# Gepetto/mpc-interface

Measured on AMD Instinct MI355X. Metric: QP assemblies/sec (P,q,G,h), biped N=16 batched, higher is better.
Workload: dtype f64; 1 GPU; C2 biped LIPM N=16 no=36 nc=76, per-instance (A,B)/given/aim, K1 on chip; batch_per_gpu=4096, global_batch=4096, streams=2

## Files before the change

mpc-interface_amd/csrc/resident.hip:

```cpp
#ifdef __HIPCC_RTC__
using __hip_internal::int32_t;
using __hip_internal::int64_t;
using __hip_internal::uint32_t;
using __hip_internal::uint64_t;
typedef unsigned long uintptr_t;
#else
#include <hip/hip_runtime.h>
#include <stdint.h>
#endif

#include "device_prims.h"
#include "plan_dev.h"
#ifdef MPCASM_SPEC
#include "plan_spec.h"
#endif
#ifndef __HIPCC_RTC__
#include "kernels.h"
#endif

namespace mpcasm {

#ifndef __HIPCC_RTC__
extern int g_phase_mask;
extern int g_resident_per_cu;
#endif

namespace {

constexpr int NT = RS_NT;
constexpr int MW = RS_NW;
constexpr int WT = NT - MW * 64;
constexpr int AXMAX = RS_AXMAX;
constexpr int RR_WORDS = RS_RR_WORDS;
constexpr int RR_COMPACT = 4;
static_assert(RS_DIAG_MAX == 2, "the per-column diagonal table holds two terms");

__host__ __device__ inline int even_up_i(int x) { return (x + 1) & ~1; }

constexpr int GU = 6;
template <class PlanT>
__host__ __device__ inline int resident_g_mode(const PlanT& p) {
  if (p.csc_gnnz != 0 || p.csc_pnnz != 0) return 3;
  if (!p.rr_packed) return 0;
  return p.rs_ngdesc != 0 ? 2 : 1;
}
static_assert(GU == RS_GDESC_PIECES && WT == RS_GDESC_THREADS, "descriptor table of G");

template <class PlanT>
__host__ __device__ inline int resident_v_doubles(const PlanT& p) {
  return (p.rs_vrow0 + p.rtot) * p.rs_ldv + 16;
}

struct ResidentLayout {
  int v, pl, ql, dvec, dcoef, dpar, img, ab, streams, ints, total_doubles;
  int ldp;
  int p_direct;
  int i_rr, i_meta, i_wtrip, i_split, i_lti, i_abmeta, i_gdesc, i_gfix, i_rrwin, i_cscp;
};

template <class PlanT>
__host__ __device__ inline ResidentLayout resident_layout(const PlanT& p) {
  ResidentLayout L;
  L.ldp = even_up_i(p.no);
  int o = 0;
  L.v = o;      o += resident_v_doubles(p);
  L.pl = o;
  L.ql = o;     o += L.ldp;
  L.dvec = o;   o += 2 * L.ldp;
  L.dcoef = o;  o += RS_DIAG_MAX * L.ldp;
  L.dpar = o;   o += RS_DIAG_MAX * L.ldp;
  L.img = o;    o += 2 * p.rs_img;
  L.ab = o;     o += 2 * p.rs_ab;
  L.streams = o; o += 2 * (MAX_SOURCES + 3);
  L.ints = o;
  int i = 0;
  L.i_rr = i;    i += p.nc * (p.rr_packed ? RR_COMPACT : RR_WORDS);
  L.i_meta = i;  i += p.rs_nchunk * 64 * 2;
  L.i_abmeta = i; i += p.rs_ab * 2 * 2;
  L.i_gdesc = i;  i += resident_g_mode(p) == 2 ? GU * WT * 2 : (resident_g_mode(p) == 3 ? 2 * p.csc_gnnz : 0);
  L.i_gfix = i;   i += resident_g_mode(p) == 2 && p.rs_ngfix != 0 ? 2 * WT : 0;
  L.i_rrwin = i;  i += p.rs_compact ? p.nc : 0;
  L.i_cscp = i;   i += resident_g_mode(p) == 3 ? p.csc_pnnz : 0;
  L.i_wtrip = i; i += RS_WAVES * 2;
  L.i_split = i; i += p.rs_nsplit;
  L.i_lti = i;   i += p.rs_nlti * RS_LTI_WORDS;
  o += even_up_i(i) / 2;
  L.p_direct = p.rs_p_direct;
  L.pl = o;
  if (!L.p_direct) o += p.no * L.ldp;
  L.total_doubles = o;
  return L;
}

__device__ __forceinline__ void dma16(const void* gsrc, unsigned lds_base) {
  unsigned keep;
  asm volatile(
      "s_mov_b32 %0, m0\n\ts_mov_b32 m0, %2\n\ts_nop 0\n\tglobal_load_lds_dwordx4 %1, off\n\t"
      "s_mov_b32 m0, %0"
      : "=&s"(keep)
      : "v"(gsrc), "s"(lds_base)
      : "memory");
}
__device__ __forceinline__ void dma4(const void* gsrc, unsigned lds_base) {
  unsigned keep;
  asm volatile(
      "s_mov_b32 %0, m0\n\ts_mov_b32 m0, %2\n\ts_nop 0\n\tglobal_load_lds_dword %1, off\n\t"
      "s_mov_b32 m0, %0"
      : "=&s"(keep)
      : "v"(gsrc), "s"(lds_base)
      : "memory");
}
__device__ __forceinline__ void dma_wait() { asm volatile("s_waitcnt vmcnt(0)" ::: "memory"); }
__device__ __forceinline__ void dma_wait_but(int later) {
  switch (later) {
    case 1: asm volatile("s_waitcnt vmcnt(1)" ::: "memory"); break;
    case 2: asm volatile("s_waitcnt vmcnt(2)" ::: "memory"); break;
    case 3: asm volatile("s_waitcnt vmcnt(3)" ::: "memory"); break;
    case 4: asm volatile("s_waitcnt vmcnt(4)" ::: "memory"); break;
    default: asm volatile("s_waitcnt vmcnt(0)" ::: "memory"); break;
  }
}

__device__ __forceinline__ int resident_trip_row(int lk) { return ((lk & 1) << 3) | ((lk & 2) << 1); }

#ifdef MPCASM_SPEC
struct TripState {
  const char* Vlane;
  const char* prc;
  double *Pl, *ql;
  int ldpl;
  bool mirror;
  const double* dvec;
  int lx, lg, lk;
  const char *ap, *bp;
  int bi, bj;
  bool isq, live;
  double acc, sum;
};

template <int I>
__device__ __forceinline__ void spec_trip(TripState& s) {
  using PC = spec::PlanConst;
  constexpr int A = spec::TRIPS[I][RT_A], B = spec::TRIPS[I][RT_B], D = spec::TRIPS[I][RT_D];
  constexpr int W = spec::TRIPS[I][RT_W], AIM = spec::TRIPS[I][RT_AIM], WORD = spec::TRIPS[I][RT_WORD];
  constexpr int BI = spec::TRIPS[I][RT_BI], BJ = spec::TRIPS[I][RT_BJ];
  constexpr int row_bytes = PC::rs_ldv * 8, ldp = (PC::no + 1) & ~1;
  constexpr int qmask = (WORD >> RT_QMASK) & 15, livemask = (WORD >> RT_LIVE) & 15;
  constexpr bool nop = (WORD >> RT_NOP) & 1, half = (WORD >> RT_HALF) & 1;
  if constexpr ((WORD >> RT_FIRST) & 1) {
    int lg_ = s.lg;
    asm volatile("" : "+v"(lg_));
    s.bi = (BI >> (8 * lg_)) & 255;
    s.bj = (BJ >> (8 * lg_)) & 255;
    s.isq = (qmask >> lg_) & 1;
    s.live = (livemask >> lg_) & 1;
    s.ap = s.Vlane + s.bi * 32;
    s.bp = s.Vlane + (s.isq ? 0 : s.bj * 32);
    s.acc = 0.0;
  }
  if constexpr ((WORD & 31) != 0) {
    const char* bsrc = qmask == 0 ? s.bp + B : (qmask == livemask ? s.bp + D : s.bp + (s.isq ? D : B));
    if constexpr (!((WORD >> RT_SHORT) & 1)) {
      constexpr int span = 3 * row_bytes;
      constexpr int AH = A + span < 65536 ? 0 : A, DH = D + span < 65536 ? 0 : D, BH = B + span < 65536 ? 0 : B;
      const unsigned pa = (unsigned)(uintptr_t)s.ap + AH;
      if constexpr (qmask == 0) {
        s.sum = mfma_trip16<A - AH, B - BH, row_bytes>(pa, (unsigned)(uintptr_t)s.bp + BH, s.sum);
      } else if constexpr (qmask == livemask) {
        s.sum = mfma_trip16<A - AH, D - DH, row_bytes>(pa, (unsigned)(uintptr_t)s.bp + DH, s.sum);
      } else {
        s.sum = mfma_trip16<A - AH, B - BH, row_bytes>(pa, (unsigned)(uintptr_t)s.bp + BH + (s.isq ? D - B : 0), s.sum);
      }
    } else {
      const int short_shift = (s.lk - resident_trip_row(s.lk)) * row_bytes;
      const double a = *reinterpret_cast<const double*>(s.ap + (A + short_shift));
      const double b = *reinterpret_cast<const double*>(bsrc + short_shift);
      s.sum = mfma_f64_4x4x4(a, b, s.sum);
    }
    if constexpr ((WORD >> RT_TERM_END) & 1) {
      const double w = *reinterpret_cast<const double*>(s.prc + W);
      if constexpr (qmask != 0 || nop) {
        const double aim = *reinterpret_cast<const double*>(s.prc + AIM);
        const double ws = half ? 0.5 * w : w;
        const double ones = quad_broadcast<1>(s.sum);
        const double m = s.isq ? ws : (nop ? 0.0 : w);
        s.acc = fma(m, fma(-(s.isq ? aim : 0.0), ones, s.sum), s.acc);
      } else {
        s.acc = fma(w, s.sum, s.acc);
      }
      s.sum = 0.0;
    }
  }
  if constexpr ((WORD >> RT_LAST) & 1) {
    int lk_ = s.lk, lx_ = s.lx;
    asm volatile("" : "+v"(lk_), "+v"(lx_));
    const int row = 4 * s.bi + lk_, col = 4 * s.bj + lx_;
    if (s.live && row < PC::no) {
      if (s.isq) {
        if (lx_ == 0) s.ql[row] = s.acc + s.dvec[ldp + row];
      } else if (col < PC::no) {
        const double val = s.acc + (row == col ? s.dvec[col] : 0.0);
        s.Pl[row * s.ldpl + col] = val;
        if (PC::rs_sym && s.bi != s.bj) s.Pl[col * s.ldpl + row] = val;
      }
    }
  }
}

struct LaneSrc {
  const char* base;
  long long stride;
  bool isg;
  int2 entry;
};
static_assert(FS_MAX == 8 && FS_WORDS == 6 && RS_LTI_MAX == 4 && RS_LTI_WORDS == 8, "plan_spec.h, as jit.hip writes it");
template <bool AB, int K>
constexpr int spec_fetch_runs() {
  if constexpr (AB)
    return K < spec::PlanConst::rs_ab / 32 ? spec::FSEG_AB_N[K] : 0;
  else
    return K < spec::PlanConst::rs_nchunk ? spec::FSEG_IMG_N[K] : 0;
}
template <bool AB, int K, int S>
__device__ __forceinline__ void spec_lane_run(LaneSrc& out, int lane, const SrcTable& src, const double* params,
                                              const double* given, const double* plan_dtab) {
  using PC = spec::PlanConst;
  if constexpr (S < spec_fetch_runs<AB, K>()) {
    constexpr int first = AB ? spec::FSEG_AB[K][S][FS_FIRST] : spec::FSEG_IMG[K][S][FS_FIRST];
    constexpr int lanes = AB ? spec::FSEG_AB[K][S][FS_LANES] : spec::FSEG_IMG[K][S][FS_LANES];
    constexpr int stream = AB ? spec::FSEG_AB[K][S][FS_STREAM] : spec::FSEG_IMG[K][S][FS_STREAM];
    constexpr int byte0 = AB ? spec::FSEG_AB[K][S][FS_BYTE] : spec::FSEG_IMG[K][S][FS_BYTE];
    constexpr int step = AB ? spec::FSEG_AB[K][S][FS_STEP] : spec::FSEG_IMG[K][S][FS_STEP];
    constexpr int period = AB ? spec::FSEG_AB[K][S][FS_PERIOD] : spec::FSEG_IMG[K][S][FS_PERIOD];
    static_assert(period >= lanes || (period & (period - 1)) == 0, "a periodic run repeats every 1, 2 or 4 lanes");
    const char* base;
    long long stride;
    if constexpr (stream < PC::nsrc) {
      base = reinterpret_cast<const char*>(src.ptr[stream]);
      stride = src.stride[stream] * (long long)sizeof(double);
    } else if constexpr (stream == PC::nsrc) {
      base = reinterpret_cast<const char*>(given);
      stride = (long long)PC::ng * (long long)sizeof(double);
    } else if constexpr (stream == PC::nsrc + 1) {
      base = reinterpret_cast<const char*>(params);
      stride = (long long)PC::nparams * (long long)sizeof(double);
    } else {
      base = reinterpret_cast<const char*>(plan_dtab + PC::doff_rs_const);
      stride = 0;
    }
    const int rel = lane - first;
    const int off = byte0 + (period < lanes ? rel & (period - 1) : rel) * step;
    if (S == 0 || lane >= first) {
      out.base = base + off;
      out.stride = stride;
      out.isg = stream == PC::nsrc;
      out.entry = int2{stream, off};
    }
    spec_lane_run<AB, K, S + 1>(out, lane, src, params, given, plan_dtab);
  }
}
template <bool AB, int K>
__device__ __forceinline__ LaneSrc spec_lane_src(int lane, const SrcTable& src, const double* params,
                                                 const double* given, const double* plan_dtab) {
  LaneSrc out{nullptr, 0, false, int2{0, 0}};
  spec_lane_run<AB, K, 0>(out, lane, src, params, given, plan_dtab);
  return out;
}
template <bool AB, int K>
__device__ __forceinline__ void spec_write_table(int2* table, int lane, const SrcTable& src, const double* params,
                                                 const double* given, const double* plan_dtab) {
  if constexpr (K < (AB ? spec::PlanConst::rs_ab / 32 : spec::PlanConst::rs_nchunk)) {
    table[K * 64 + lane] = spec_lane_src<AB, K>(lane, src, params, given, plan_dtab).entry;
    spec_write_table<AB, K + 1>(table, lane, src, params, given, plan_dtab);
  }
}
template <int K>
__device__ __forceinline__ void spec_first_ab(int lane, long inst0, long inst1, bool two, unsigned ab_lds,
                                              const SrcTable& src, const double* params, const double* given,
                                              const double* plan_dtab) {
  using PC = spec::PlanConst;
  if constexpr (K < PC::rs_ab / 32) {
    const LaneSrc m = spec_lane_src<true, K>(lane, src, params, given, plan_dtab);
    dma4(m.base + inst0 * m.stride, ab_lds + (unsigned)(K * 32 * 8));
    if (two) dma4(m.base + inst1 * m.stride, ab_lds + (unsigned)((PC::rs_ab + K * 32) * 8));
    spec_first_ab<K + 1>(lane, inst0, inst1, two, ab_lds, src, params, given, plan_dtab);
  }
}
template <int K>
__device__ __forceinline__ void spec_first_image(int lane, long inst, long ginst, unsigned img_lds, const SrcTable& src,
                                                 const double* params, const double* given, const double* plan_dtab) {
  using PC = spec::PlanConst;
  if constexpr (K < PC::rs_nchunk && K < 32) {
    if constexpr (spec_fetch_runs<false, K>() != 0) {
      const LaneSrc m = spec_lane_src<false, K>(lane, src, params, given, plan_dtab);
      const char* a = m.base + (m.isg ? ginst : inst) * m.stride;
      if constexpr (PC::rs_unit == 16)
        dma16(a, img_lds + (unsigned)(K * 64 * 16));
      else
        dma4(a, img_lds + (unsigned)(K * 64 * 4));
    }
    spec_first_image<K + 1>(lane, inst, ginst, img_lds, src, params, given, plan_dtab);
  }
}
constexpr bool spec_ab_by_runs() {
  for (int k = 0; k < spec::PlanConst::rs_ab / 32; ++k)
    if (spec::FSEG_AB_N[k] == 0) return false;
  return true;
}

template <int I, int N>
__device__ __forceinline__ void spec_trips(TripState& s) {
  if constexpr (I < N) {
    spec_trip<I>(s);
    __builtin_amdgcn_sched_barrier(0);
    spec_trips<I + 1, N>(s);
  }
}
template <int WAVE>
__device__ __forceinline__ void spec_wave_trips(TripState& s) {
  spec_trips<spec::WTRIP[WAVE][0], spec::WTRIP[WAVE][0] + spec::WTRIP[WAVE][1]>(s);
}
#endif

template <int JC, bool STAMPS, bool GEN, class PlanT>
__device__ __forceinline__ void resident_body(
    const PlanT& p, const int32_t* __restrict__ plan_itab, const double* __restrict__ plan_dtab,
    const SrcTable& src, const double* __restrict__ params, const double* __restrict__ given,
    double* __restrict__ P, double* __restrict__ q, double* __restrict__ G,
    double* __restrict__ h, int batch, int phases, unsigned long long* __restrict__ stamps) {
  extern __shared__ __attribute__((aligned(16))) double lds[];
  const int tid = threadIdx.x, lane = tid & 63;
  const int wave = __builtin_amdgcn_readfirstlane(tid >> 6);
  unsigned long long t_acc[8] = {0, 0, 0, 0, 0, 0, 0, 0}, t_prev = 0;
  const unsigned long long t_begin = STAMPS ? __builtin_amdgcn_s_memtime() : 0;
#define SETUP_STAMP(k)                                                                  \
  if (STAMPS && stamps != nullptr && lane == 0)                                         \
    stamps[((size_t)gridDim.x + blockIdx.x) * (NT / 64) * 8 + wave * 8 + (k)] =         \
        __builtin_amdgcn_s_memtime() - t_begin;
  const bool stamping = STAMPS && stamps != nullptr;
#define MPCASM_STAMP(slot)                                         \
  if (STAMPS && stamping) {                                        \
    const unsigned long long t_now = __builtin_amdgcn_s_memtime(); \
    t_acc[slot] += t_now - t_prev;                                 \
    t_prev = t_now;                                                \
  }
  const ResidentLayout L = resident_layout(p);
  const int no = p.no, nc = p.nc, ldv = p.rs_ldv, vd = p.rs_vd, ldp = L.ldp;

  double* V = lds + L.v;
  double* Pl = lds + L.pl;
  double* ql = lds + L.ql;
  double* dvec = lds + L.dvec;
  double2* dcoef = reinterpret_cast<double2*>(lds + L.dcoef);
  int4* dpar = reinterpret_cast<int4*>(lds + L.dpar);
  double* strm = lds + L.streams;
  int* itb = reinterpret_cast<int*>(lds + L.ints);
  int* rr = itb + L.i_rr;
  int2* meta = reinterpret_cast<int2*>(itb + L.i_meta);
  int* wtrip = itb + L.i_wtrip;
  int* split = itb + L.i_split;
  int* lti = itb + L.i_lti;
  int2* abmeta = reinterpret_cast<int2*>(itb + L.i_abmeta);
  int2* gdesc = reinterpret_cast<int2*>(itb + L.i_gdesc);
  int2* gfix = reinterpret_cast<int2*>(itb + L.i_gfix);
  int* rrwin = itb + L.i_rrwin;
  const unsigned img_lds = (unsigned)(uintptr_t)(lds + L.img);
  const int unit = p.rs_unit, nchunk = p.rs_nchunk;
  const int lx = lane & 3, lg = (lane >> 2) & 3, lk = lane >> 4;
  const unsigned ab_lds = (unsigned)(uintptr_t)(lds + L.ab);
  auto fetch_ab = [&](long inst, int slot) {
    for (int k = 0; k < p.rs_ab / 32; ++k) {
      const int2 m = abmeta[k * 64 + lane];
      const char* base = reinterpret_cast<const char* const*>(strm)[2 * m.x];
      const long long stride = reinterpret_cast<const long long*>(strm)[2 * m.x + 1];
      dma4(base + inst * stride + m.y,
           __builtin_amdgcn_readfirstlane(ab_lds + (unsigned)((slot * p.rs_ab + k * 32) * 8)));
    }
  };
  auto generate_sources = [&](int buf, int slot) {
    double* im = lds + L.img + buf * p.rs_img;
    const double* ab = lds + L.ab + slot * p.rs_ab;
    auto generate = [&](auto word) __attribute__((always_inline)) {
      const int n = word(LT_N), m = word(LT_M);
      const int N = word(LT_HORIZON), nn = n * n, nm = n * m;
      const double* Am = ab + word(LT_A);
      const double* Bm = ab + word(LT_B);
      double* TA = im + word(LT_TA);
      double* TB = im + word(LT_TB);
      double* TP = im + word(LT_TP);
      if (n <= 4 && n + m <= 4) {
        int lane_ = lane;
#ifdef MPCASM_SPEC
        asm volatile("" : "+v"(lane_));
#endif
        const int grp = lane_ >> 4, gi = lane_ & 3, gc = (lane_ >> 2) & 3;
        const bool live = gi < n && gc < n + m;
        double ar[4];
#pragma unroll
        for (int t = 0; t < 4; ++t) ar[t] = gi < n && t < n ? Am[gi * n + t] : 0.0;
        double x = !live ? 0.0 : (gc < m ? Bm[gi * m + gc] : Am[gi * n + (gc - m)]);
        double* out = gc < m ? TB + gi * m + gc : TA + gi * n + (gc - m);
        const int step = gc < m ? nm : nn;
        auto advance = [&]() {
          double y = ar[0] * quad_broadcast<0>(x);
          y = fma(ar[1], quad_broadcast<1>(x), y);
          y = fma(ar[2], quad_broadcast<2>(x), y);
          y = fma(ar[3], quad_broadcast<3>(x), y);
          x = y;
        };
        const int head = N < 4 ? N : 4;
        for (int d = 0; d < head; ++d) {
          if (live && grp == 0) out[d * step] = x;
          advance();
        }
        if (N > 4) {
          asm volatile("s_waitcnt lgkmcnt(0)" ::: "memory");
#pragma unroll
          for (int t = 0; t < 4; ++t) ar[t] = gi < n && t < n ? TA[3 * nn + gi * n + t] : 0.0;
          x = live ? out[grp * step] : 0.0;
          for (int d = grp + 4; d - grp < N; d += 4) {
            advance();
            if (live && d < N) out[d * step] = x;
          }
        }
        return;
      }
      for (int e = lane; e < nn; e += 64) {
        const double v = Am[e];
        TA[e] = v;
        TP[e] = v;
      }
      for (int e = lane; e < nm; e += 64) TB[e] = Bm[e];
      asm volatile("s_waitcnt lgkmcnt(0)" ::: "memory");
      int have = 1;
      for (int s_ = 0; have < N; ++s_) {
        const double* Pw = TP + s_ * nn;
        const int cnt = have < N - have ? have : N - have;
        const int na = cnt * nn, nb = cnt * nm, total = na + nb + nn;
        for (int e = lane; e < total; e += 64) {
          const double* X;
          double* out;
          int w, r;
          if (e < na) {
            const int d = e / nn;
            r = e - d * nn;
            X = TA + d * nn, out = TA + (have + d) * nn, w = n;
          } else if (e < na + nb) {
            const int d = (e - na) / nm;
            r = (e - na) - d * nm;
            X = TB + d * nm, out = TB + (have + d) * nm, w = m;
          } else {
            r = e - na - nb;
            X = Pw, out = TP + (s_ + 1) * nn, w = n;
          }
          const int i = r / w, j = r - i * w;
          double acc = 0.0;
          for (int t = 0; t < n; ++t) acc = fma(Pw[i * n + t], X[t * w + j], acc);
          out[r] = acc;
        }
        asm volatile("s_waitcnt lgkmcnt(0)" ::: "memory");
        have += cnt;
      }
    };
#ifdef MPCASM_SPEC
    if constexpr (PlanT::rs_nlti > 0) generate([](int k) { return spec::LTI[0][k]; });
    if constexpr (PlanT::rs_nlti > 1) generate([](int k) { return spec::LTI[1][k]; });
    if constexpr (PlanT::rs_nlti > 2) generate([](int k) { return spec::LTI[2][k]; });
    if constexpr (PlanT::rs_nlti > 3) generate([](int k) { return spec::LTI[3][k]; });
#else
    for (int g = 0; g < p.rs_nlti; ++g) {
      const int* rec = lti + g * RS_LTI_WORDS;
      generate([&](int k) { return __builtin_amdgcn_readfirstlane(rec[k]); });
    }
#endif
  };
  const int run_over = (phases >> 10) & 7;
  const int run_shift = run_over ? run_over : ((long)batch >= 16L * gridDim.x && !(phases & 256) ? 2 : 0);
  const unsigned vblock = (phases & 8192) && gridDim.x % 8 == 0
                              ? (blockIdx.x % 8) * (gridDim.x / 8) + blockIdx.x / 8 : blockIdx.x;
  auto instance_at = [&](int n) -> long {
    return ((((long)(n >> run_shift) * gridDim.x + vblock)) << run_shift) + (n & ((1 << run_shift) - 1));
  };
  const bool gen = GEN && p.rs_nlti != 0;
  const int ct = tid - 64, CT = NT - 64;
#ifdef MPCASM_SPEC
  constexpr int ZK = 2;
#else
  constexpr int ZK = 0;
#endif
  int v_zb[ZK > 0 ? ZK : 1];
  const int zt0 = tid >= MW * 64 ? tid - MW * 64 : tid + WT;
#pragma unroll
  for (int k = 0; k < ZK; ++k) {
    const int e = zt0 + k * NT;
    v_zb[k] = L.p_direct && e < p.rs_nzblk * 8 ? (plan_itab + p.off_rs_zblk)[e >> 3] : 0;
  }
  int c_sg[JC], c_dst[JC];
  double c_coef[JC];
  auto load_program = [&]() __attribute__((always_inline)) {
    const int4* prog = reinterpret_cast<const int4*>(plan_itab + p.off_rs_prog);
#pragma unroll
    for (int j = 0; j < JC; ++j) {
      const bool have = j < p.rs_jc;
      const int4 w = have ? prog[j * NT + tid] : int4{0, -1, 0, 0};
      c_sg[j] = w.x;
      c_dst[j] = w.y;
      c_coef[j] = __hiloint2double(w.w, w.z);
    }
  };
#ifdef MPCASM_SPEC
  constexpr int FK = JC <= 5 ? 3 : 0;
#else
  constexpr int FK = 0;
#endif
  const int32_t* gix = src.stride[MAX_SOURCES - 1] == -1
                           ? reinterpret_cast<const int32_t*>(src.ptr[MAX_SOURCES - 1]) : nullptr;
  const char* f_base[FK > 0 ? FK : 1];
  int f_stride[FK > 0 ? FK : 1];
  bool f_isg[FK > 0 ? FK : 1];
  bool f_shared[FK > 0 ? FK : 1];
  bool f_fast = FK > 0;
#ifdef MPCASM_SPEC
  constexpr bool prog_early = true;
#else
  constexpr bool prog_early = false;
#endif
  auto prepare_fetch = [&]() __attribute__((always_inline)) {
    if (FK > 0 && wave < MW) {
#pragma unroll
      for (int j = 0; j < FK; ++j) {
        const int k = wave + j * MW;
        const int2 m = meta[(k < nchunk ? k : 0) * 64 + lane];
        const long long stride = reinterpret_cast<const long long*>(strm)[2 * m.x + 1];
        f_base[j] = reinterpret_cast<const char* const*>(strm)[2 * m.x] + m.y;
        f_stride[j] = (int)stride;
        f_isg[j] = m.x == p.nsrc;
        f_shared[j] = __all(stride == 0);
        f_fast = f_fast && stride >= 0 && stride < (1ll << 31);
      }
    }
    f_fast = __builtin_amdgcn_readfirstlane(__all(f_fast));
  };
  auto fetch_image = [&](long inst, int buf, bool settled) {
    const unsigned dst0 = img_lds + (unsigned)buf * (unsigned)p.rs_img * 8u;
    const long ginst = gix != nullptr ? (long)gix[inst] : inst;
    int kfirst = wave;
    if (FK > 0 && f_fast) {
#pragma unroll
      for (int j = 0; j < FK; ++j) {
        const int k = wave + j * MW;
        if (k < nchunk && !(settled && f_shared[j])) {
          const char* a = f_base[j] + (unsigned long long)(f_isg[j] ? ginst : inst) * (unsigned)f_stride[j];
          const unsigned dst = __builtin_amdgcn_readfirstlane(dst0 + (unsigned)(k * 64 * unit));
          if (unit == 16)
            dma16(a, dst);
          else
            dma4(a, dst);
        }
      }
      kfirst = wave + FK * MW;
    }
    for (int k = kfirst; k < nchunk; k += MW) {
      const int2 m = meta[k * 64 + lane];
      const char* base = reinterpret_cast<const char* const*>(strm)[2 * m.x];
      const long long stride = reinterpret_cast<const long long*>(strm)[2 * m.x + 1];
      if (settled && __all(stride == 0)) continue;
      const char* a = base + (m.x == p.nsrc ? ginst : inst) * stride + m.y;
      const unsigned dst = __builtin_amdgcn_readfirstlane(dst0 + (unsigned)(k * 64 * unit));
      if (unit == 16)
        dma16(a, dst);
      else
        dma4(a, dst);
    }
  };
  if (wave == 0) {
    constexpr int MK = 2;
#ifdef MPCASM_SPEC
    constexpr int nltw = 0;
#else
    const int nltw = p.rs_nlti * RS_LTI_WORDS;
#endif
    const int nab2 = p.rs_ab * 2, nmeta = nchunk * 64;
    const int2* t_ab = reinterpret_cast<const int2*>(plan_itab + p.off_rs_abmeta);
    const int2* t_meta = reinterpret_cast<const int2*>(plan_itab + p.off_rs_inmeta);
    const int32_t* t_lti = plan_itab + p.off_rs_lti;
    int2 v_ab = int2{0, 0}, v_meta[MK];
    int v_lti = 0;
#ifdef MPCASM_SPEC
    constexpr bool ab_runs = spec_ab_by_runs();
    constexpr unsigned on_table = spec::FSEG_IMG_TABLE;
    constexpr bool img_runs = on_table == 0 && PlanT::rs_nchunk <= 32;
    constexpr int img_late = __builtin_popcount(on_table) + (PlanT::rs_nchunk > 32 ? PlanT::rs_nchunk - 32 : 0);
    const int ab_later = ab_runs ? nchunk : img_late;
    if (gen && ab_runs) {
      const long i1 = instance_at(1);
      spec_first_ab<0>(lane, instance_at(0), i1, i1 < batch, __builtin_amdgcn_readfirstlane(ab_lds), src, params,
                       given, plan_dtab);
    }
    if (ab_runs) SETUP_STAMP(2)
    {
      const long inst = instance_at(0), ginst = gix != nullptr ? (long)gix[inst] : inst;
      spec_first_image<0>(lane, inst, ginst, __builtin_amdgcn_readfirstlane(img_lds), src, params, given, plan_dtab);
    }
#else
    constexpr bool ab_runs = false, img_runs = false;
    constexpr unsigned on_table = ~0u;
    const int ab_later = nchunk;
#endif
    if (!ab_runs && lane < nab2) v_ab = t_ab[lane];
    if (lane < nltw) v_lti = t_lti[lane];
    if (!img_runs) {
#pragma unroll
      for (int k = 0; k < MK; ++k) v_meta[k] = lane + k * 64 < nmeta ? t_meta[lane + k * 64] : int2{0, 0};
    }
    if (prog_early) load_program();
    if (!ab_runs) {
      if (lane < nab2) abmeta[lane] = v_ab;
      for (int i = lane + 64; i < nab2; i += 64) abmeta[i] = t_ab[i];
    }
    if (lane < nltw) lti[lane] = v_lti;
    for (int i = lane + 64; i < nltw; i += 64) lti[i] = t_lti[i];
    if (!img_runs) {
#pragma unroll
      for (int k = 0; k < MK; ++k)
        if (lane + k * 64 < nmeta) meta[lane + k * 64] = v_meta[k];
      for (int i = lane + MK * 64; i < nmeta; i += 64) meta[i] = t_meta[i];
    }
#ifdef MPCASM_SPEC
    if constexpr (ab_runs) spec_write_table<true, 0>(abmeta, lane, src, params, given, plan_dtab);
    if constexpr (img_runs) spec_write_table<false, 0>(meta, lane, src, params, given, plan_dtab);
#endif
    for (int t = 0; t < p.nsrc + 3; ++t) {
      const int s = t - p.nsrc;
      const double* base = s < 0 ? src.ptr[t]
                                 : (s == 0 ? given : (s == 1 ? params : plan_dtab + p.doff_rs_const));
      const long long stride =
          s < 0 ? src.stride[t] : (s == 0 ? (long long)p.ng : (s == 1 ? (long long)p.nparams : 0));
      if (lane == 0) {
        reinterpret_cast<const double**>(strm)[2 * t] = base;
        reinterpret_cast<long long*>(strm)[2 * t + 1] = stride * (long long)sizeof(double);
      }
    }
    if (gen && !ab_runs) {
      fetch_ab(instance_at(0), 0);
      if (instance_at(1) < batch) fetch_ab(instance_at(1), 1);
    }
    if (!ab_runs) SETUP_STAMP(2)
    if (!img_runs) {
      const long inst = instance_at(0), ginst = gix != nullptr ? (long)gix[inst] : inst;
      for (int k = 0; k < nchunk; ++k) {
        if (k < 32 && !((on_table >> k) & 1)) continue;
        const int2 m = meta[k * 64 + lane];
        const char* base = reinterpret_cast<const char* const*>(strm)[2 * m.x];
        const long long stride = reinterpret_cast<const long long*>(strm)[2 * m.x + 1];
        const char* a = base + (m.x == p.nsrc ? ginst : inst) * stride + m.y;
        const unsigned dst = __builtin_amdgcn_readfirstlane(img_lds + (unsigned)(k * 64 * unit));
        if (unit == 16)
          dma16(a, dst);
        else
          dma4(a, dst);
      }
    }
    SETUP_STAMP(0)
    lds_barrier();
    SETUP_STAMP(1)
    prepare_fetch();
    SETUP_STAMP(3)
    if (gen) {
      dma_wait_but(ab_later);
      SETUP_STAMP(4)
      generate_sources(0, 0);
    }
    if (!prog_early) load_program();
    SETUP_STAMP(5)
  } else {
    SETUP_STAMP(0)
    lds_barrier();
    SETUP_STAMP(1)
    prepare_fetch();
    SETUP_STAMP(2)
    load_program();
    typedef int i32x4 __attribute__((ext_vector_type(4)));
    typedef int i32x2 __attribute__((ext_vector_type(2)));
    typedef double f64x2 __attribute__((ext_vector_type(2)));
    constexpr int RRK = 3;
    const int32_t* trr = plan_itab + p.off_rs_rr;
    const int nrr = p.rr_packed ? 0 : nc * RR_WORDS;
    int v_rr[RRK], v_wtrip = 0, v_split = 0, v_rrwin = 0;
    int2 v_gd[GU], v_gfix = int2{0, 0};
    i32x4 v_dpar = {0, 0, 0, 0};
    i32x2 v_rrc = {0, 0}, v_rrp = {0, 0};
    int v_rre = 0;
    f64x2 v_dcoef = {0.0, 0.0};
    const bool own_gd = resident_g_mode(p) == 2 && tid >= MW * 64;
    const bool own_diag = p.ndiag != 0 && ct >= 0 && ct < no;
    const int wt_ = tid - MW * 64;
    if (own_diag) {
      v_dpar = reinterpret_cast<const i32x4*>(plan_itab + p.off_rs_dpar)[ct];
      v_dcoef = reinterpret_cast<const f64x2*>(plan_dtab + p.doff_rs_dcoef)[ct];
    }
    if (ct >= 0) {
#pragma unroll
      for (int k = 0; k < RRK; ++k) v_rr[k] = ct + k * CT < nrr ? trr[ct + k * CT] : 0;
      if (ct < RS_WAVES * 2) v_wtrip = (plan_itab + p.off_rs_wtrip)[ct];
      if (ct < p.rs_nsplit) v_split = (plan_itab + p.off_rs_split)[ct];
      if (p.rr_packed && ct < nc) {
        v_rrc = *reinterpret_cast<const i32x2*>(trr + ct * RR_WORDS + RR_CENTER);
        v_rre = trr[ct * RR_WORDS + RR_EXTREME];
        v_rrp = *reinterpret_cast<const i32x2*>(trr + ct * RR_WORDS + RR_PACKED);
      }
      if (p.rs_compact && ct < nc) v_rrwin = (plan_itab + p.off_rs_rrwin)[ct];
    }
    if (own_gd) {
      const int2* gd = reinterpret_cast<const int2*>(plan_itab + p.off_rs_gdesc);
#pragma unroll
      for (int u = 0; u < GU; ++u) v_gd[u] = gd[u * WT + wt_];
      if (p.rs_ngfix != 0) v_gfix = reinterpret_cast<const int2*>(plan_itab + p.off_rs_gfix)[wt_];
    }
    if (ct >= 0) {
      if (!L.p_direct)
        for (int i = ct; i < no * ldp; i += CT) Pl[i] = 0.0;
      double2* V2 = reinterpret_cast<double2*>(V);
      const int n2 = resident_v_doubles(p) / 2;
      for (int i = ct; i < n2; i += CT) V2[i] = double2{0.0, 0.0};
      for (int i = ct; i < 2 * ldp; i += CT) dvec[i] = 0.0;
#pragma unroll
      for (int k = 0; k < RRK; ++k)
        if (ct + k * CT < nrr) rr[ct + k * CT] = v_rr[k];
      for (int i = ct + RRK * CT; i < nrr; i += CT) rr[i] = trr[i];
      if (p.rs_compact) {
        if (ct < nc) rrwin[ct] = v_rrwin;
        for (int R = ct + CT; R < nc; R += CT) rrwin[R] = (plan_itab + p.off_rs_rrwin)[R];
      }
      if (p.rr_packed) {
        static_assert(RR_CENTER == 8 && RR_EXTREME == 13 && RR_PACKED == 14, "the row record's second half");
        if (ct < nc)
          reinterpret_cast<int4*>(rr)[ct] = int4{v_rrp.x, v_rrp.y, v_rrc.x | (v_rrc.y << 16), v_rre};
        for (int R = ct + CT; R < nc; R += CT) {
          const int32_t* g = trr + R * RR_WORDS;
          reinterpret_cast<int4*>(rr)[R] =
              int4{g[RR_PACKED], g[RR_PACKED + 1], g[RR_CENTER] | (g[RR_CENTER + 1] << 16), g[RR_EXTREME]};
        }
      }
      if (resident_g_mode(p) == 3) {
        const int2* cg = reinterpret_cast<const int2*>(plan_itab + p.off_csc_g);
        for (int i = ct; i < p.csc_gnnz; i += CT) gdesc[i] = cg[i];
        for (int i = ct; i < p.csc_pnnz; i += CT) (itb + L.i_cscp)[i] = (plan_itab + p.off_csc_p)[i];
      }
      if (ct < RS_WAVES * 2) wtrip[ct] = v_wtrip;
      if (ct < p.rs_nsplit) split[ct] = v_split;
      for (int i = ct + CT; i < p.rs_nsplit; i += CT) split[i] = (plan_itab + p.off_rs_split)[i];
    }
    if (own_gd) {
#pragma unroll
      for (int u = 0; u < GU; ++u) gdesc[u * WT + wt_] = v_gd[u];
      if (p.rs_ngfix != 0) gfix[wt_] = v_gfix;
    }
    if (own_diag) {
      dpar[ct] = int4{v_dpar.x, v_dpar.y, v_dpar.z, v_dpar.w};
      dcoef[ct] = double2{v_dcoef.x, v_dcoef.y};
    }
    SETUP_STAMP(3)
    SETUP_STAMP(4)
    SETUP_STAMP(5)
  }
  lds_barrier();
  SETUP_STAMP(6)
  for (int r = tid; r < p.rtot; r += NT) V[(p.rs_vrow0 + r) * ldv + vd + 1] = 1.0;

  const bool lookahead = (phases & 128) != 0;
  if (wave == 0) dma_wait();
  SETUP_STAMP(7)

  const int wt = tid - MW * 64;
  const int npair = no >> 1;
  const int gtotal = nc * npair;
  const int g_mode = resident_g_mode(p);
  int zoff[ZK > 0 ? ZK : 1];
#pragma unroll
  for (int k = 0; k < ZK; ++k) {
    const int e = zt0 + k * NT;
    zoff[k] = -1;
    if (L.p_direct && e < p.rs_nzblk * 8) {
      const int z = v_zb[k], row = 4 * (z >> 8) + ((e >> 1) & 3), col = 4 * (z & 255) + 2 * (e & 1);
      if (row < no && col < no)
        zoff[k] = (row * no + col) | (col + 1 < no ? ((no & 1) == 0 ? 1 << 30 : 1 << 29) : 0);
    }
  }
  const bool skew = !(phases & 16384);
  const int g_rot = skew && gtotal % 8 == 0 && gtotal > 0 ? (int)((blockIdx.x * 53u) % (unsigned)(gtotal / 8)) * 8 : 0;
  const int g_e0 = wt >= 0 && gtotal > 0 ? (wt + g_rot) % gtotal : 0;
  const int g_first = wt >= 0 && npair > 0 ? ((g_e0 / npair) << 16) | (g_e0 % npair) : 0;
  const int g_dR = npair > 0 ? WT / npair : 0, g_dcp = npair > 0 ? WT % npair : 0;


  const auto g_packed = [&](double* Gb, const double* V, const double* prm) __attribute__((always_inline)) {
    double2* G2 = reinterpret_cast<double2*>(Gb);
    int first = g_first;
    asm volatile("" : "+v"(first));
    int R = first >> 16, cp = first & 0xFFFF;
    for (int e0 = wt; e0 < gtotal; e0 += 3 * WT) {
      int2 ds[3];
      int c2[3], wn[3], at[3];
#pragma unroll
      for (int u = 0; u < 3; ++u) {
        const int Rr = e0 + u * WT < gtotal ? R : 0;
        ds[u] = *reinterpret_cast<const int2*>(rr + Rr * RR_COMPACT);
        wn[u] = p.rs_compact ? rrwin[Rr] : 0;
        c2[u] = 2 * cp;
        at[u] = Rr * npair + cp;
        cp += g_dcp;
        R += g_dR;
        if (cp >= npair) {
          cp -= npair;
          ++R;
        }
        if (R >= nc) R -= nc;
      }
      double a0[3], a1[3];
      double2 v0[3], v1[3];
      if (p.rs_compact) {
#pragma unroll
        for (int u = 0; u < 3; ++u) {
          const unsigned win = (unsigned)wn[u], cpair = (unsigned)c2[u] >> 1;
          const unsigned d0 = cpair - (win & 255), d1 = cpair - ((win >> 16) & 255);
          const bool in0 = d0 < ((win >> 8) & 255), in1 = d1 < (win >> 24);
          a0[u] = prm[in0 ? ds[u].y & 0xFFFF : p.nparams];
          a1[u] = prm[in1 ? (unsigned)ds[u].y >> 16 : p.nparams];
          v0[u] = *reinterpret_cast<const double2*>(V + (ds[u].x & 0xFFFF) + (in0 ? 2 * d0 : 0));
          v1[u] = *reinterpret_cast<const double2*>(V + ((unsigned)ds[u].x >> 16) + (in1 ? 2 * d1 : 0));
        }
      } else {
#pragma unroll
        for (int u = 0; u < 3; ++u) {
          a0[u] = prm[ds[u].y & 0xFFFF];
          a1[u] = prm[(unsigned)ds[u].y >> 16];
          v0[u] = *reinterpret_cast<const double2*>(V + (ds[u].x & 0xFFFF) + c2[u]);
          v1[u] = *reinterpret_cast<const double2*>(V + ((unsigned)ds[u].x >> 16) + c2[u]);
        }
      }
#pragma unroll
      for (int u = 0; u < 3; ++u) {
        const int e = e0 + u * WT;
        double2 r;
        r.x = fma(a1[u], v1[u].x, a0[u] * v0[u].x);
        r.y = fma(a1[u], v1[u].y, a0[u] * v0[u].y);
        if (e < gtotal) store_result(&G2[at[u]], r);
      }
    }
  };

  if (STAMPS && stamping) t_prev = __builtin_amdgcn_s_memtime();
  int buf = 0, iter = 0;
  for (long inst = instance_at(0); inst < batch; inst = instance_at(iter + 1), buf ^= 1, ++iter) {
    const double* img = lds + L.img + buf * p.rs_img;
    const double* prm = img + p.rs_img_params;
    lds_barrier();
    MPCASM_STAMP(0)

    auto compose = [&]() {
      if (p.ndiag != 0) {
        int c = tid;
        asm volatile("" : "+v"(c));
        if (c < no) {
          const int4 par = dpar[c];
          const double2 co = dcoef[c];
          const double w0 = prm[par.x], a0 = prm[par.y], w1 = prm[par.z], a1 = prm[par.w];
          dvec[c] = (w0 * co.x) * co.x + (w1 * co.y) * co.y;
          dvec[ldp + c] = w0 * (co.x * (0.0 - a0)) + w1 * (co.y * (0.0 - a1));
        }
      }
      if (phases & 1) {
        double va[JC], vg[JC];
  #pragma unroll
        for (int j = 0; j < JC; ++j) {
          va[j] = img[c_sg[j] & 0xFFFF];
          vg[j] = img[(unsigned)c_sg[j] >> 16];
        }
        double acc = 0.0;
  #pragma unroll
        for (int j = 0; j < JC; ++j) {
          acc += c_coef[j] * va[j] * vg[j];
          if (c_dst[j] >= 0) {
            if (c_dst[j] & RS_DST_ACC)
              __hip_atomic_fetch_add(&V[c_dst[j] & ~RS_DST_ACC], acc, __ATOMIC_RELAXED,
                                     __HIP_MEMORY_SCOPE_WORKGROUP);
            else
              V[c_dst[j]] = acc;
          }
          acc = c_dst[j] >= 0 ? 0.0 : acc;
        }
      }
    };
    const long nxt = instance_at(iter + 1), nxt2 = instance_at(iter + 2);
    if (wave < MW) {
      compose();
      lds_barrier();
      MPCASM_STAMP(1)
      __builtin_amdgcn_s_setprio(2);
      if (lookahead && nxt < batch && (phases & 16)) fetch_image(nxt, buf ^ 1, iter >= 1);
      if (wave == 0 && (GEN && p.rs_nlti != 0) && nxt2 < batch) fetch_ab(nxt2, buf);
      MPCASM_STAMP(7)
      if (wave == MW - 1 && (GEN && p.rs_nlti != 0) && nxt < batch) generate_sources(buf ^ 1, buf ^ 1);
    } else {
      compose();
      lds_barrier();
      MPCASM_STAMP(1)
      if (G != nullptr && (phases & 8)) {
        double* Gb = G + (size_t)inst * nc * no;
        if (g_mode == 3) {
          double* Gd = G + (size_t)inst * p.csc_gnnz;
          int w_ = wt;
          asm volatile("" : "+v"(w_));
          for (int e0 = w_; e0 < p.csc_gnnz; e0 += 3 * WT) {
            int2 ds[3];
#pragma unroll
            for (int u = 0; u < 3; ++u) ds[u] = gdesc[min(e0 + u * WT, p.csc_gnnz - 1)];
            double a0[3], a1[3], v0[3], v1[3];
#pragma unroll
            for (int u = 0; u < 3; ++u) {
              a0[u] = prm[ds[u].y & 0xFFFF];
              v0[u] = V[ds[u].x & 0xFFFF];
              if (!p.csc_gsingle) {
                a1[u] = prm[(unsigned)ds[u].y >> 16];
                v1[u] = V[(unsigned)ds[u].x >> 16];
              }
            }
#pragma unroll
            for (int u = 0; u < 3; ++u)
              if (e0 + u * WT < p.csc_gnnz)
                Gd[e0 + u * WT] = p.csc_gsingle ? a0[u] * v0[u] : fma(a1[u], v1[u], a0[u] * v0[u]);
          }
        } else if (g_mode == 2) {
          double2* G2 = reinterpret_cast<double2*>(Gb);
          int wt_ = wt;
          asm volatile("" : "+v"(wt_));
          const bool all_single = p.rs_gsingle == (1 << (GU * (WT / 64))) - 1;
#ifdef MPCASM_SPEC
          constexpr int GB = spec::PlanConst::rs_gsingle == (1 << (GU * (WT / 64))) - 1 ? GU : 3;
#else
          constexpr int GB = 3;
#endif
          static_assert(GU % GB == 0, "batches of pieces");
          const bool h_mine = wt_ < nc;
          int fix_u = RS_GFIX_NONE;
          double fa1 = 0.0;
          double2 fv1{0.0, 0.0};
          int2 fd{0, 0};
          if (p.rs_ngfix != 0) fd = gfix[wt_];
          const int4 hc4 = reinterpret_cast<const int4*>(rr)[h_mine ? wt_ : 0];
          const int4 hr = int4{0, hc4.w, hc4.x, hc4.y};
          const int2 hc = int2{hc4.z & 0xFFFF, (int)((unsigned)hc4.z >> 16)};
          double ha0 = 0.0, ha1 = 0.0, hc0 = 0.0, hc1 = 0.0, hd0 = 0.0, hd1 = 0.0, hext = 0.0;
#pragma unroll
          for (int u0 = 0; u0 < GU; u0 += GB) {
            int2 ds[GB];
#pragma unroll
            for (int u = 0; u < GB; ++u) ds[u] = gdesc[(u0 + u) * WT + wt_];
            if (u0 == 0 && p.rs_ngfix != 0) {
              fix_u = (unsigned)fd.x >> 16;
              fa1 = prm[fd.y];
              fv1 = *reinterpret_cast<const double2*>(V + (fd.x & 0xFFFF));
            }
            if (u0 == 0) {
              ha0 = prm[hr.w & 0xFFFF];
              ha1 = prm[(unsigned)hr.w >> 16];
              hc0 = prm[hc.x];
              hc1 = prm[hc.y];
              hd0 = V[(hr.z & 0xFFFF) + vd];
              hd1 = V[((unsigned)hr.z >> 16) + vd];
              hext = prm[hr.y];
            }
            double a0[GB], a1[GB];
            double2 v0[GB], v1[GB];
            bool one[GB];
#pragma unroll
            for (int u = 0; u < GB; ++u) {
              one[u] = all_single || ((p.rs_gsingle >> ((u0 + u) * (WT / 64) + (wave - MW))) & 1);
              a0[u] = prm[ds[u].y & 0xFFFF];
              v0[u] = *reinterpret_cast<const double2*>(V + (ds[u].x & 0xFFFF));
              if (!one[u]) {
                a1[u] = prm[(unsigned)ds[u].y >> 16];
                v1[u] = *reinterpret_cast<const double2*>(V + ((unsigned)ds[u].x >> 16));
              }
            }
#pragma unroll
            for (int u = 0; u < GB; ++u) {
              const int e = wt_ + (u0 + u) * WT;
              double2 r;
              if (one[u]) {
                r.x = a0[u] * v0[u].x;
                r.y = a0[u] * v0[u].y;
                if (p.rs_ngfix != 0 && u0 + u == fix_u) {
                  r.x = fma(fa1, fv1.x, r.x);
                  r.y = fma(fa1, fv1.y, r.y);
                }
              } else {
                r.x = fma(a1[u], v1[u].x, a0[u] * v0[u].x);
                r.y = fma(a1[u], v1[u].y, a0[u] * v0[u].y);
              }
              if (e < gtotal && !((phases & 512) && r.x == r.x))
                store_result(&G2[e], r);
            }
            if (u0 == 0 && h_mine) {
              double ac = ha0 * hc0, ad = ha0 * hd0;
              ac += ha1 * hc1;
              ad = fma(ha1, hd1, ad);
              (h + (size_t)inst * nc)[wt_] = (hext + ac) - ad;
            }
          }
        } else if (g_mode == 1) {
          g_packed(Gb, V, prm);
        } else if ((no & 1) == 0) {
          int w_ = wt;
          asm volatile("" : "+v"(w_));
          const int dR = WT / npair, dcp = WT - dR * npair;
          int e = w_, R = w_ / npair, cp = w_ - (w_ / npair) * npair;
          double2* G2 = reinterpret_cast<double2*>(Gb);
          while (e < gtotal) {
            const int* rec = rr + R * RR_WORDS;
            const int naxes = rec[RR_NAXES];
            double2 accv{0.0, 0.0};
            for (int ax = 0; ax < naxes; ++ax) {
              const double a = prm[rec[RR_ARROW + ax]];
              const double2 v = *reinterpret_cast<const double2*>(V + rec[RR_VOFF + ax] + 2 * cp);
              accv.x = fma(a, v.x, accv.x);
              accv.y = fma(a, v.y, accv.y);
            }
            store_result(&G2[e], accv);
            e += WT;
            cp += dcp;
            R += dR;
            if (cp >= npair) {
              cp -= npair;
              ++R;
            }
          }
        } else {
          int w_ = wt;
          asm volatile("" : "+v"(w_));
          const int total = nc * no;
          const int dR = WT / no, dc = WT - dR * no;
          int e = w_, R = w_ / no, c = w_ - (w_ / no) * no;
          while (e < total) {
            const int* rec = rr + R * RR_WORDS;
            const int naxes = rec[RR_NAXES];
            double accv = 0.0;
            for (int ax = 0; ax < naxes; ++ax)
              accv = fma(prm[rec[RR_ARROW + ax]], V[rec[RR_VOFF + ax] + c], accv);
            store_result(&Gb[e], accv);
            e += WT;
            c += dc;
            R += dR;
            if (c >= no) {
              c -= no;
              ++R;
            }
          }
        }
        double* hb = h + (size_t)inst * nc;
        int Rh = g_mode == 2 ? wt + WT : wt;
        asm volatile("" : "+v"(Rh));
        for (int R = Rh; R < nc; R += WT) {
          if (p.rr_packed) {
            const int4 c = reinterpret_cast<const int4*>(rr)[R];
            const double a0 = prm[c.y & 0xFFFF], a1 = prm[(unsigned)c.y >> 16];
            double ac = a0 * prm[c.z & 0xFFFF], ad = a0 * V[(c.x & 0xFFFF) + vd];
            ac += a1 * prm[(unsigned)c.z >> 16];
            ad = fma(a1, V[((unsigned)c.x >> 16) + vd], ad);
            hb[R] = (prm[c.w] + ac) - ad;
            continue;
          }
          const int* rec = rr + R * RR_WORDS;
          const int naxes = rec[RR_NAXES];
          double ac = 0.0, ad = 0.0;
          for (int ax = 0; ax < naxes; ++ax) {
            const double a = prm[rec[RR_ARROW + ax]];
            ac += a * prm[rec[RR_CENTER + ax]];
            ad = fma(a, V[rec[RR_VOFF + ax] + vd], ad);
          }
          hb[R] = (prm[rec[RR_EXTREME]] + ac) - ad;
        }
      }
      MPCASM_STAMP(3)
      __builtin_amdgcn_s_setprio(2);
    }
#ifdef MPCASM_SPEC
    if (P != nullptr && (phases & 2)) {
      static_assert(RS_WAVES == 8, "one case per wavefront");
      TripState st;
      st.Vlane = reinterpret_cast<const char*>(V) + resident_trip_row(lk) * (ldv * 8) + lx * 8;
      st.prc = reinterpret_cast<const char*>(prm);
      st.Pl = L.p_direct ? P + (size_t)inst * no * no : Pl;
      st.ldpl = L.p_direct ? no : ldp;
      st.ql = ql;
      st.dvec = dvec;
      st.lx = lx, st.lg = lg, st.lk = lk;
      st.ap = st.bp = st.Vlane;
      st.bi = st.bj = 0;
      st.isq = st.live = false;
      st.acc = st.sum = 0.0;
      switch (wave) {
        case 0: spec_wave_trips<0>(st); break;
        case 1: spec_wave_trips<1>(st); break;
        case 2: spec_wave_trips<2>(st); break;
        case 3: spec_wave_trips<3>(st); break;
        case 4: spec_wave_trips<4>(st); break;
        case 5: spec_wave_trips<5>(st); break;
        case 6: spec_wave_trips<6>(st); break;
        default: spec_wave_trips<7>(st); break;
      }
    }
#else
    if (P != nullptr && (phases & 2)) {
      const int t0 = __builtin_amdgcn_readfirstlane(wtrip[2 * wave]);
      const int tn = __builtin_amdgcn_readfirstlane(wtrip[2 * wave + 1]);
      typedef int i32x8 __attribute__((ext_vector_type(8)));
      typedef const __attribute__((address_space(4))) i32x8* const_i32x8_ptr;
      const_i32x8_ptr tg = (const_i32x8_ptr)(uintptr_t)(plan_itab + p.off_rs_trip) + t0;
      if (tn > 0) {
        const char* prc = reinterpret_cast<const char*>(prm);
        const int row_bytes = ldv * (int)sizeof(double);
        const int short_shift = (lk - resident_trip_row(lk)) * row_bytes;
        const char* Vlane = reinterpret_cast<const char*>(V) + resident_trip_row(lk) * row_bytes + lx * 8;
        const char *ap = Vlane, *bp = Vlane;
        int bi = 0, bj = 0;
        bool isq = false, live = false;
        i32x8 rn = tg[0];
        double acc = 0.0, sum = 0.0;
        for (int t = 0; t < tn; ++t) {
          const i32x8 r = rn;
          rn = tg[t + 1];
          const int word = r[RT_WORD];
          if ((word >> RT_FIRST) & 1) {
            bi = (r[RT_BI] >> (8 * lg)) & 255;
            bj = (r[RT_BJ] >> (8 * lg)) & 255;
            isq = (word >> (RT_QMASK + lg)) & 1;
            live = (word >> (RT_LIVE + lg)) & 1;
            ap = Vlane + bi * 32;
            bp = Vlane + (isq ? 0 : bj * 32);
            acc = 0.0;
          }
          if (word & 31) {
            const int boff = isq ? r[RT_D] : r[RT_B];
            if (!((word >> RT_SHORT) & 1)) {
              sum = mfma_trip16_at((unsigned)(uintptr_t)(ap + r[RT_A]), (unsigned)(uintptr_t)(bp + boff),
                                   (unsigned)row_bytes, sum);
            } else {
              const double a = *reinterpret_cast<const double*>(ap + (r[RT_A] + short_shift));
              const double b = *reinterpret_cast<const double*>(bp + (boff + short_shift));
              sum = mfma_f64_4x4x4(a, b, sum);
            }
            if ((word >> RT_TERM_END) & 1) {
              const double w = *reinterpret_cast<const double*>(prc + r[RT_W]);
              if (word & ((15 << RT_QMASK) | (1 << RT_NOP))) {
                const double aim = *reinterpret_cast<const double*>(prc + r[RT_AIM]);
                const double ws = (word >> RT_HALF) & 1 ? 0.5 * w : w;
                const double ones = quad_broadcast<1>(sum);
                const double m = isq ? ws : ((word >> RT_NOP) & 1 ? 0.0 : w);
                acc = fma(m, fma(-(isq ? aim : 0.0), ones, sum), acc);
              } else {
                acc = fma(w, sum, acc);
              }
              sum = 0.0;
            }
          }
          if ((word >> RT_LAST) & 1) {
            const int row = 4 * bi + lk, col = 4 * bj + lx;
            if (live && row < no) {
              if (isq) {
                if (lx == 0) ql[row] = acc + dvec[ldp + row];
              } else if (col < no) {
                const double val = acc + (row == col ? dvec[col] : 0.0);
                double* Pout = L.p_direct ? P + (size_t)inst * no * no : Pl;
                const int ldo = L.p_direct ? no : ldp;
                Pout[row * ldo + col] = val;
                if (p.rs_sym && bi != bj) Pout[col * ldo + row] = val;
              }
            }
          }
        }
      }
    }
#endif
    MPCASM_STAMP(2)
    __builtin_amdgcn_s_setprio(0);
    lds_barrier();
    MPCASM_STAMP(4)

    if (wave < MW) {
      if (!lookahead && nxt < batch && (phases & 16)) fetch_image(nxt, buf ^ 1, iter >= 1);
      dma_wait();
      for (int i = tid; i < p.rs_nsplit; i += MW * 64) V[split[i]] = 0.0;
    }
    MPCASM_STAMP(5)
    if (P != nullptr && (phases & 32)) {
      double* Pb = P + (size_t)inst * no * no;
      int t_ = tid >= MW * 64 ? tid - MW * 64 : tid + WT;
      asm volatile("" : "+v"(t_));
      if (L.p_direct) {
#pragma unroll
        for (int k = 0; k < ZK; ++k)
          if (zoff[k] >= 0) {
            double* z = Pb + (zoff[k] & 0xFFFFFF);
            if (zoff[k] & (1 << 30))
              *reinterpret_cast<double2*>(z) = double2{0.0, 0.0};
            else {
              z[0] = 0.0;
              if (zoff[k] & (1 << 29)) z[1] = 0.0;
            }
          }
        const int32_t* zb = plan_itab + p.off_rs_zblk;
        for (int e = t_ + ZK * NT; e < p.rs_nzblk * 8; e += NT) {
          const int z = zb[e >> 3], row = 4 * (z >> 8) + ((e >> 1) & 3), col = 4 * (z & 255) + 2 * (e & 1);
          if (row < no && col < no) {
            if (col + 1 < no && ((no & 1) == 0))
              *reinterpret_cast<double2*>(Pb + (size_t)row * no + col) = double2{0.0, 0.0};
            else {
              Pb[(size_t)row * no + col] = 0.0;
              if (col + 1 < no) Pb[(size_t)row * no + col + 1] = 0.0;
            }
          }
        }
      } else if (g_mode == 3) {
        double* Pd = P + (size_t)inst * p.csc_pnnz;
        const int* cp = itb + L.i_cscp;
        for (int e = t_; e < p.csc_pnnz; e += NT) Pd[e] = Pl[cp[e]];
      } else if ((no & 1) == 0) {
        const int total = no * npair;
        double2* P2 = reinterpret_cast<double2*>(Pb);
        const double2* Pl2 = reinterpret_cast<const double2*>(Pl);
        const int rot = skew && total % 8 == 0 ? (int)((blockIdx.x * 37u) % (unsigned)(total / 8)) * 8 : 0;
        for (int e = t_; e < total; e += NT) {
          const int at = e + rot < total ? e + rot : e + rot - total;
          store_result(&P2[at], Pl2[at]);
        }
      } else {
        for (int e = t_; e < no * no; e += NT) {
          const int row = e / no;
          store_result(&Pb[e], Pl[row * ldp + (e - row * no)]);
        }
      }
      double* qb = q + (size_t)inst * no;
      for (int c = t_; c < no; c += NT) qb[c] = ql[c];
    }
    MPCASM_STAMP(6)
  }
  if (STAMPS && stamping && lane == 0) {
#pragma unroll
    for (int i = 0; i < 8; ++i) stamps[((size_t)blockIdx.x * (NT / 64) + wave) * 8 + i] = t_acc[i];
  }
#undef MPCASM_STAMP
#undef SETUP_STAMP
}

#ifdef MPCASM_SPEC
}
#ifndef MPCASM_SPEC_WAVES_PER_EU
#define MPCASM_SPEC_WAVES_PER_EU 4
#endif
extern "C" __global__ __launch_bounds__(RS_NT, MPCASM_SPEC_WAVES_PER_EU) void resident_spec_kernel(
    const int32_t* __restrict__ plan_itab, const double* __restrict__ plan_dtab, SrcTable src,
    const double* __restrict__ params, const double* __restrict__ given, double* __restrict__ P,
    double* __restrict__ q, double* __restrict__ G, double* __restrict__ h, int batch, int phases,
    unsigned long long* __restrict__ stamps) {
  constexpr spec::PlanConst p{};
#ifdef MPCASM_SPEC_STAMPS
  constexpr bool stamped = true;
#else
  constexpr bool stamped = false;
#endif
#ifdef MPCASM_SPEC_PHASES
  const int mask = MPCASM_SPEC_PHASES;
#else
  const int mask = phases;
#endif
  resident_body<spec::JC, stamped, spec::PlanConst::rs_nlti != 0>(p, plan_itab, plan_dtab, src, params,
                                                               given, P, q, G, h, batch, mask, stamps);
}
namespace {
#else
template <int JC, bool STAMPS, bool GEN>
__global__ __launch_bounds__(NT, 4) void resident_assemble_kernel(
    PlanDev p, SrcTable src, const double* __restrict__ params, const double* __restrict__ given,
    double* __restrict__ P, double* __restrict__ q, double* __restrict__ G,
    double* __restrict__ h, int batch, int phases, unsigned long long* __restrict__ stamps) {
  resident_body<JC, STAMPS, GEN>(p, p.itab, p.dtab, src, params, given, P, q, G, h, batch, phases,
                                 stamps);
}
#endif

#ifndef __HIPCC_RTC__

template <int JC>
int launch_jc(const PlanDev& p, const SrcTable& src, const double* params, const double* given,
              double* P, double* q, double* G, double* h, void* work, int batch, size_t lds_bytes,
              int num_cus, hipStream_t stream, hipError_t* err) {
  auto kernel = (g_phase_mask & 64) ? resident_assemble_kernel<JC, true, true>
                : p.rs_nlti != 0    ? resident_assemble_kernel<JC, false, true>
                                    : resident_assemble_kernel<JC, false, false>;
  struct Residency {
    int device;
    size_t lds;
    int per_cu;
  };
  constexpr int KEPT = 8;
  static thread_local Residency kept[3][KEPT];
  static thread_local int nkept[3] = {0, 0, 0};
  const int slot = (g_phase_mask & 64) ? 2 : (p.rs_nlti != 0 ? 1 : 0);
  int device = 0;
  (void)hipGetDevice(&device);
  int found = -1;
  for (int i = 0; i < nkept[slot]; ++i)
    if (kept[slot][i].device == device && kept[slot][i].lds == lds_bytes) found = kept[slot][i].per_cu;
  if (found < 0) {
    if (lds_bytes > 64 * 1024) {
      *err = allow_whole_lds(reinterpret_cast<const void*>(kernel));
      if (*err != hipSuccess) return MPCASM_ERR_HIP;
    }
    int n = 0;
    *err = hipOccupancyMaxActiveBlocksPerMultiprocessor(&n, kernel, NT, lds_bytes);
    if (*err != hipSuccess) return MPCASM_ERR_HIP;
    found = n;
    const int at = nkept[slot] < KEPT ? nkept[slot]++ : (int)(lds_bytes % KEPT);
    kept[slot][at] = Residency{device, lds_bytes, n};
  }
  int per_cu = found;
  if (per_cu < 1) return MPCASM_ERR_LIMIT;
  if (t_per_cu > 0 && t_per_cu < per_cu) per_cu = t_per_cu;
  long grid = (long)num_cus * per_cu;
  if (t_grid > 0 && t_grid < grid) grid = t_grid;
  if (grid > batch) grid = batch;
  hipLaunchKernelGGL(kernel, dim3((unsigned)grid), dim3(NT), lds_bytes, stream, p, src, params,
                     given, P, q, G, h, batch, g_phase_mask,
                     (g_phase_mask & 64) ? static_cast<unsigned long long*>(work) : nullptr);
  *err = hipGetLastError();
  return *err == hipSuccess ? MPCASM_OK : MPCASM_ERR_HIP;
}
#endif

}

#ifndef __HIPCC_RTC__
int resident_choose_p_direct(const PlanDev& p, int option) {
  PlanDev q = p;
  q.rs_p_direct = 0;
  const bool fits = (size_t)resident_layout(q).total_doubles * sizeof(double) <= (size_t)RESIDENT_LDS_LIMIT;
  return (!fits || option == 1) ? 1 : (option == 2 ? 0 : 2);
}

int resident_p_direct_for(const PlanDev& p, int batch) {
  if (p.rs_p_direct != 2) return p.rs_p_direct;
  PlanDev q = p;
  q.rs_p_direct = 0;
  const size_t with_p = (size_t)resident_layout(q).total_doubles * sizeof(double);
  q.rs_p_direct = 1;
  const size_t without = (size_t)resident_layout(q).total_doubles * sizeof(double);
  constexpr size_t HALF_CU = 80 * 1024;
  const double per_instance = 8.0 * ((double)p.no * p.no + p.no + (double)p.nc * p.no + p.nc);
  if (with_p > HALF_CU && without <= HALF_CU && per_instance < 128.0 * 1024) return 1;
  return per_instance * batch < 560e6 ? 1 : 0;
}

size_t resident_lds_bytes(const PlanDev& p) {
  if (!p.rs_ok || p.rs_jc > RS_JC_MAX || p.no > WT || p.no < 1 || p.max_axes > AXMAX) return 0;
  if ((long)(p.rs_vrow0 + p.rtot) * p.rs_ldv > (1 << 20)) return 0;
  return (size_t)resident_layout(p).total_doubles * sizeof(double);
}

bool resident_inputs_aligned(const PlanDev& p, const SrcTable& src, const double* params,
                             const double* given) {
  if (p.rs_unit != 16) return true;
  auto ok = [](const void* base, long long stride) {
    return (reinterpret_cast<uintptr_t>(base) & 15) == 0 && (stride & 1) == 0;
  };
  for (int s = 0; s < p.nsrc; ++s)
    if (((p.rs_src16 >> s) & 1) && !ok(src.ptr[s], src.stride[s])) return false;
  return ok(given, p.ng) && ok(params, p.nparams);
}

int launch_assemble_resident(const PlanDev& p, const SrcTable& src, const double* params,
                             const double* given, double* P, double* q, double* G, double* h,
                             void* work, int batch, size_t lds_bytes, int num_cus,
                             hipStream_t stream, hipError_t* err) {
#define MPCASM_RS_ARGS p, src, params, given, P, q, G, h, work, batch, lds_bytes, num_cus, stream, err
  if (p.rs_jc <= 3) return launch_jc<3>(MPCASM_RS_ARGS);
  if (p.rs_jc <= 4) return launch_jc<4>(MPCASM_RS_ARGS);
  if (p.rs_jc <= 5) return launch_jc<5>(MPCASM_RS_ARGS);
  if (p.rs_jc <= 8) return launch_jc<8>(MPCASM_RS_ARGS);
  return launch_jc<RS_JC_MAX>(MPCASM_RS_ARGS);
#undef MPCASM_RS_ARGS
}
#endif

}
```

Measured before the change: 172.9 million assemblies/s.

## Deepen image prefetch to two instances ahead in resident kernel

When lookahead is on, the setup phase now preloads the second instance's image into the other LDS buffer. Each iteration then issues the image fetch for instance iter+2 into the current buffer after it has been consumed, rather than fetching iter+1 right after compose. The gix lookup for the instance two ahead is hoisted before compose and broadcast with readfirstlane, and the A/B fetch is moved to the same late slot. This is meant to give DMA a full iteration to complete so the dma_wait no longer stalls. In exchange the setup does more work, and the buffer reuse depends on the added waits being ordered correctly, which adds a risk of races.

```diff
diff --git a/mpc-interface_amd/csrc/resident.hip b/mpc-interface_amd/csrc/resident.hip
--- a/mpc-interface_amd/csrc/resident.hip
+++ b/mpc-interface_amd/csrc/resident.hip
@@ -541,9 +541,8 @@
     }
     f_fast = __builtin_amdgcn_readfirstlane(__all(f_fast));
   };
-  auto fetch_image = [&](long inst, int buf, bool settled) {
+  auto fetch_image = [&](long inst, long ginst, int buf, bool settled) {
     const unsigned dst0 = img_lds + (unsigned)buf * (unsigned)p.rs_img * 8u;
-    const long ginst = gix != nullptr ? (long)gix[inst] : inst;
     int kfirst = wave;
     if (FK > 0 && f_fast) {
 #pragma unroll
@@ -661,13 +660,29 @@
           dma4(a, dst);
       }
     }
+    const bool second = (phases & 128) && (phases & 16) && instance_at(1) < batch;
+    if (second) {
+      const long inst = instance_at(1), ginst = gix != nullptr ? (long)gix[inst] : inst;
+      const unsigned dst0 = img_lds + (unsigned)p.rs_img * 8u;
+      for (int k = 0; k < nchunk; ++k) {
+        const int2 m = meta[k * 64 + lane];
+        const char* base = reinterpret_cast<const char* const*>(strm)[2 * m.x];
+        const long long stride = reinterpret_cast<const long long*>(strm)[2 * m.x + 1];
+        const char* a = base + (m.x == p.nsrc ? ginst : inst) * stride + m.y;
+        const unsigned dst = __builtin_amdgcn_readfirstlane(dst0 + (unsigned)(k * 64 * unit));
+        if (unit == 16)
+          dma16(a, dst);
+        else
+          dma4(a, dst);
+      }
+    }
     SETUP_STAMP(0)
     lds_barrier();
     SETUP_STAMP(1)
     prepare_fetch();
     SETUP_STAMP(3)
     if (gen) {
-      dma_wait_but(ab_later);
+      dma_wait_but(ab_later + (second ? nchunk : 0));
       SETUP_STAMP(4)
       generate_sources(0, 0);
     }
@@ -893,15 +908,18 @@
       }
     };
     const long nxt = instance_at(iter + 1), nxt2 = instance_at(iter + 2);
+    long g_next2 = nxt2;
     if (wave < MW) {
+      int g_ahead = 0;
+      if (gix != nullptr && lookahead && wave < nchunk && nxt2 < batch) g_ahead = gix[nxt2];
       compose();
       lds_barrier();
       MPCASM_STAMP(1)
       __builtin_amdgcn_s_setprio(2);
-      if (lookahead && nxt < batch && (phases & 16)) fetch_image(nxt, buf ^ 1, iter >= 1);
-      if (wave == 0 && (GEN && p.rs_nlti != 0) && nxt2 < batch) fetch_ab(nxt2, buf);
+      if ((lookahead && wave < nchunk) || (wave == MW - 1 && gen)) dma_wait();
+      if (gix != nullptr) g_next2 = (long)__builtin_amdgcn_readfirstlane(g_ahead);
       MPCASM_STAMP(7)
-      if (wave == MW - 1 && (GEN && p.rs_nlti != 0) && nxt < batch) generate_sources(buf ^ 1, buf ^ 1);
+      if (wave == MW - 1 && gen && nxt < batch) generate_sources(buf ^ 1, buf ^ 1);
     } else {
       compose();
       lds_barrier();
@@ -1189,8 +1207,15 @@
     MPCASM_STAMP(4)
 
     if (wave < MW) {
-      if (!lookahead && nxt < batch && (phases & 16)) fetch_image(nxt, buf ^ 1, iter >= 1);
-      dma_wait();
+      if (phases & 16) {
+        if (lookahead) {
+          if (nxt2 < batch) fetch_image(nxt2, g_next2, buf, true);
+        } else if (nxt < batch) {
+          fetch_image(nxt, gix != nullptr ? (long)gix[nxt] : nxt, buf ^ 1, iter >= 1);
+        }
+      }
+      if (wave == MW - 1 && gen && nxt2 < batch) fetch_ab(nxt2, buf);
+      if (!lookahead) dma_wait();
       for (int i = tid; i < p.rs_nsplit; i += MW * 64) V[split[i]] = 0.0;
     }
     MPCASM_STAMP(5)
```

After: 163.8 million assemblies/s. 5.3% lower.
